# Pixie8888/R3DFSSeg

Measured on AMD Instinct MI355X. Metric: episodes/sec S3DIS 2-way 5-shot 2048-pt (MPTI+attention, train step: forward+backward+grad all-reduce+Adam), higher is better.
Workload: dtype f32 (index-free GEMMs -- self-attention, 1x1 convolutions, weight gradients, the EdgeConv backward's edge GEMMs -- as bf16x3 split products on the bf16 MFMA with fp32 accumulate; every index-deciding result: fp32)

## Files before the change

r3dfsseg_amd/csrc/knn.hip:

```cpp
#include <stdlib.h>
#include "common.h"

#define KNN_Q 32
#define KNN_CH 128
#define KNN_SLAB 64
#define KNN_ROWS_PER_WAVE 8

enum { R3D_SCORE_DGCNN = 0, R3D_SCORE_L2 = 1 };

__global__ void r3d_sqnorm_kernel(const float* __restrict__ x, long ldx, int rows, int C,
                                  float* __restrict__ out) {
  int i = blockIdx.x * blockDim.x + threadIdx.x;
  if (i >= rows) return;
  const float* p = x + (long)i * ldx;
  float acc = 0.f;
  for (int c = 0; c < C; ++c) acc = __builtin_fmaf(p[c], p[c], acc);
  out[i] = acc;
}

template <int R>
struct TopList {
  float v[R];
  int id[R];
};
// ... 342 lines not shown
    const int cbase = 32 * st;
#pragma unroll
    for (int r = 0; r < 16; ++r) {
      const float s_r = sc[r];
      unsigned long long m = __ballot(s_r >= tauq[r] && s_r > thr[r]);
      while (m) {
        unsigned lo = (unsigned)m, hi = (unsigned)(m >> 32);
        const int slo = lo ? __ffs((int)lo) - 1 : 0;
        const int shi = hi ? __ffs((int)hi) - 1 : 0;
        const float cvlo = lo ? r3d_readlane_f(s_r, slo) : -INFINITY;
        const float cvhi = hi ? r3d_readlane_f(s_r, 32 + shi) : -INFINITY;
        lo &= lo - 1;
        hi &= hi - 1;
        m = ((unsigned long long)hi << 32) | lo;
        const float cv = h ? cvhi : cvlo;
        const int cidx = cbase + (h ? shi : slo);
        const bool act = cv > thr[r];
        const unsigned long long ge = __ballot(lv[r] >= cv);
        const int p = h ? __popc((unsigned)(ge >> 32)) : __popc((unsigned)ge);
        const float upv = dpp_wave_shr1_f(lv[r]);
        const int upi = dpp_wave_shr1_i(li[r]);
        if (act) {
          if (j == p) { lv[r] = cv; li[r] = cidx; }
          else if (j > p) { lv[r] = upv; li[r] = upi; }
        }
        const float tlo = r3d_readlane_f(lv[r], klo);
        const float thi = r3d_readlane_f(lv[r], khi);
        thr[r] = h ? thi : tlo;
      }
    }
  };
  {
    int st = w;
    if (st < nsub) bload(st, bfA, njA);
    while (st < nsub) {
      const int st2 = st + 4;
      if (st2 < nsub) bload(st2, bfB, njB);
      {
        f32x16 sc;
        scores(st, bfA, njA, sc);
        select(st, sc);
      }
      st = st2;
      if (st >= nsub) break;
      const int st3 = st + 4;
      if (st3 < nsub) bload(st3, bfA, njA);
      {
        f32x16 sc;
        scores(st, bfB, njB, sc);
        select(st, sc);
      }
      st = st3;
    }
  }
  KSTAMP(3);

  __syncthreads();
  float* mv = smem;
  int* mi = (int*)(smem + 32 * 128);
#pragma unroll
  for (int r = 0; r < 16; ++r) {
    const int q = r3d_acc_row(r, lane);
    mv[(q * 4 + w) * 32 + j] = lv[r];
    mi[(q * 4 + w) * 32 + j] = li[r];
  }
  __syncthreads();
  for (int qq = 0; qq < 8; ++qq) {
    const int q = 8 * w + qq;
    const int row = q0 + q;
    if (row >= n) break;
    const float v0 = mv[q * 128 + lane], v1 = mv[q * 128 + 64 + lane];
    const int i0 = mi[q * 128 + lane], i1 = mi[q * 128 + 64 + lane];
    int rank0 = 0, rank1 = 0;
#pragma unroll
    for (int l4 = 0; l4 < 4; ++l4) {
      const float lvv = (l4 < 2) ? v0 : v1;
      const int lii = (l4 < 2) ? i0 : i1;
      const unsigned long long real = __ballot(lvv != -INFINITY);
      const int cnt = __popc((unsigned)(real >> (32 * (l4 & 1))));
      for (int t = 0; t < cnt; ++t) {
        const float ov = r3d_readlane_f(lvv, 32 * (l4 & 1) + t);
        const int oi = __builtin_amdgcn_readlane(lii, 32 * (l4 & 1) + t);
        rank0 += entry_better(ov, oi, v0, i0) ? 1 : 0;
        rank1 += entry_better(ov, oi, v1, i1) ? 1 : 0;
      }
    }
    if (v0 != -INFINITY && rank0 < k) {
      idx_out[((long)b * N + row) * k + rank0] = i0;
      if (score_out) score_out[((long)b * N + row) * k + rank0] = v0;
    }
    if (v1 != -INFINITY && rank1 < k) {
      idx_out[((long)b * N + row) * k + rank1] = i1;
      if (score_out) score_out[((long)b * N + row) * k + rank1] = v1;
    }
  }
  KSTAMP(4);
}

static __device__ __forceinline__ unsigned knn_lane_xor(unsigned v, int j, int lane) {
  const int x = (int)v;
  switch (j) {
    case 1: return (unsigned)__builtin_amdgcn_update_dpp(x, x, 0xB1, 0xF, 0xF, false);
    case 2: return (unsigned)__builtin_amdgcn_update_dpp(x, x, 0x4E, 0xF, 0xF, false);
    case 4: {
      const int t = __builtin_amdgcn_update_dpp(x, x, 0x104, 0xF, 0x5, false);
      return (unsigned)__builtin_amdgcn_update_dpp(t, x, 0x114, 0xF, 0xA, false);
    }
    case 8: return (unsigned)__builtin_amdgcn_update_dpp(x, x, 0x128, 0xF, 0xF, false);
    case 16: {
      const auto r = __builtin_amdgcn_permlane16_swap(v, v, false, false);
      return (lane & 16) ? r[0] : r[1];
    }
    default: {
      const auto r = __builtin_amdgcn_permlane32_swap(v, v, false, false);
      return (lane & 32) ? r[0] : r[1];
    }
  }
}

template <int R>
static __device__ __forceinline__ void knn_bitonic_desc(unsigned (&khi)[R], unsigned (&klo)[R], int lane) {
  static_assert(R == 1 || R == 2 || R == 4 || R == 8, "a power of two");
#pragma unroll
  for (int k = 2; k <= 64 * R; k <<= 1) {
#pragma unroll
    for (int j = k >> 1; j > 0; j >>= 1) {
      if (j >= 64) {
        const int dj = j >> 6;
#pragma unroll
        for (int i = 0; i < R; ++i) {
          if (i & dj) continue;
          const bool desc = ((64 * i) & k) == 0;
          const unsigned long long a = ((unsigned long long)khi[i] << 32) | klo[i];
          const unsigned long long b = ((unsigned long long)khi[i + dj] << 32) | klo[i + dj];
          const bool swap = desc ? a < b : a > b;
          const unsigned ah = khi[i], al = klo[i];
          khi[i] = swap ? khi[i + dj] : ah; klo[i] = swap ? klo[i + dj] : al;
          khi[i + dj] = swap ? ah : khi[i + dj]; klo[i + dj] = swap ? al : klo[i + dj];
        }
      } else {
        const bool lower = (lane & j) == 0;
#pragma unroll
        for (int i = 0; i < R; ++i) {
          const bool desc = (((64 * i) | lane) & k) == 0;
          const unsigned oh = knn_lane_xor(khi[i], j, lane), ol = knn_lane_xor(klo[i], j, lane);
          const unsigned long long a = ((unsigned long long)khi[i] << 32) | klo[i];
          const unsigned long long b = ((unsigned long long)oh << 32) | ol;
          const bool take = (lower == desc) ? b > a : b < a;
          khi[i] = take ? oh : khi[i];
          klo[i] = take ? ol : klo[i];
        }
      }
    }
  }
}

template <int KB_WAVES, int KB_CAP, int KB_TOP, int KCH ,
          int KB_SAMPLE ,
          bool FULLC ,
          int SMODE ,
          bool BFA ,
          bool BFB = false >
__global__ __launch_bounds__(64 * KB_WAVES) __attribute__((amdgpu_waves_per_eu(KB_WAVES == 4 && (FULLC || KCH < 32) ? 3 : 2)))
void r3d_knn_append_kernel(
    const float* __restrict__ xT, long ldT, int N, int C, int k, int mode, const int* __restrict__ n_dev, int n_dev_stride,
    const float* __restrict__ nrm, int* __restrict__ idx_out, float* __restrict__ score_out,
    int* __restrict__ status, int* __restrict__ tile_flags, int nsplit, int* __restrict__ idx_tmp,
    float* __restrict__ sc_tmp, const unsigned short* __restrict__ xpk ,
    const float* __restrict__ cnorm ,
    const float* __restrict__ xpm , long ldx) {
  static_assert(!BFA || (KCH == 32 && FULLC), "the bf16 threshold pass takes whole 64-channel chunks");
  static_assert(!BFB || BFA, "the bf16 filter pass shares the threshold pass's pieces");
  constexpr int KB_GROUPS = KB_WAVES * 32;
  const int z = blockIdx.z;
  extern __shared__ __attribute__((aligned(16))) float smem[];
  __shared__ int cnt_s[32];
  __shared__ float tau_s[32];
  const int lin = r3d_xcd_swizzle((int)(blockIdx.y * gridDim.x + blockIdx.x), (int)(gridDim.x * gridDim.y));
  const int b = lin / (int)gridDim.x, tile_x = lin - b * (int)gridDim.x;
  const int n = n_dev ? min(n_dev[(long)b * n_dev_stride], N) : N;
  const int q0 = tile_x * 32;
  if (q0 >= n) return;
  const int tid = threadIdx.x, lane = tid & 63, w = tid >> 6;
  const int h = lane >> 5, j = lane & 31;
  const int nch = (C + 2 * KCH - 1) / (2 * KCH);
  const int Cs = nch * 2 * KCH + (BFB ? 4 : 1);
  float* Aq = smem;
  float* region = smem + 32 * Cs;
  const float* xb = xT + (long)b * C * ldT;
  const float* nb = nrm + (long)b * N;

  for (int e = tid; e < 32 * nch * 2 * KCH; e += 64 * KB_WAVES) {
    const int c = e >> 5, jj = e & 31;
    const float v = xb[(long)min(c, C - 1) * ldT + min(q0 + jj, n - 1)];
    Aq[jj * Cs + c] = r3d_keep(v, c < C && q0 + jj < n);
  }
  if (tid < 32) cnt_s[tid] = 0;
  const int Cp = nch * 64;
  const int QRS = 2 * Cp + 8;
  unsigned short* Aqb = reinterpret_cast<unsigned short*>(region + ((32 * (KB_TOP * KB_GROUPS + 1) + 3) & ~3));
  const unsigned short* xpb = BFA ? xpk + (long)b * N * 2 * Cp : nullptr;
  if (BFA) {
    const int cpr = 2 * Cp / 8;
    for (int e = tid; e < 32 * cpr; e += 64 * KB_WAVES) {
      const int c8 = e >> 5, jj = e & 31;
      *reinterpret_cast<r3d_u32x4*>(Aqb + jj * QRS + 8 * c8) =
          *reinterpret_cast<const r3d_u32x4*>(xpb + ((long)c8 * N + min(q0 + jj, n - 1)) * 8);
    }
  }
  KSTAMP(8);
  float nq[16];
#pragma unroll
  for (int r = 0; r < 16; ++r) {
    const int row = q0 + r3d_acc_row(r, lane);
    nq[r] = r3d_keep(nb[min(row, n - 1)], row < n);
  }
  const float* cnb = BFA ? cnorm + (long)b * N : nullptr;
  const float slack = (float)(C + 8) * 0x1p-24f;
  auto bound_k = [&](int i) { return cnb[i] * (1.f + 0x1p-12f) + nb[i] * slack; };
  float* kq_s = reinterpret_cast<float*>(Aqb + 32 * QRS);
  if (BFA && tid < 32) kq_s[tid] = bound_k(min(q0 + tid, n - 1));
  auto bound_ku = [&](int i) { return cnb[i] * (1.f - 0x1p-12f) - nb[i] * slack; };
  if (BFB && tid < 32) kq_s[32 + tid] = bound_ku(min(q0 + tid, n - 1));
  __syncthreads();

  const int nsub = ((n + 31) / 32 - z + nsplit - 1) / nsplit;
  const int my_sub = (nsub - w + KB_WAVES - 1) / KB_WAVES;
  const int T = (w < nsub) ? my_sub * nch : 0;

  int stride = KB_SAMPLE;
  auto bload = [&](int t, float (&bf)[KCH]) {
    const int st = (w + KB_WAVES * stride * (t / nch)) * nsplit + z, ch = (t % nch);
    const int cand = 32 * st + j;
    const bool ok = cand < n;
    const int cc = min(cand, n - 1);
    if (FULLC) {
      const float* p = xb + (long)(2 * KCH * ch + h) * ldT + cc;
      const long st2 = 2 * ldT;
#pragma unroll
      for (int s = 0; s < KCH; ++s) bf[s] = p[s * st2];
    } else {
#pragma unroll
      for (int s = 0; s < KCH; ++s) {
        const int c = 2 * KCH * ch + 2 * s + h;
        bf[s] = r3d_keep(xb[(long)min(c, C - 1) * ldT + cc], ok && c < C);
      }
    }
  };
  f32x16 acc;
  auto mma = [&](int t, const float (&bf)[KCH]) {
    const int ch = (t % nch);
    if (ch == 0) {
#pragma unroll
      for (int r = 0; r < 16; ++r) acc[r] = 0.f;
    }
    const float* ap = Aq + j * Cs + 2 * KCH * ch + h;
    float av[KCH];
#pragma unroll
    for (int s = 0; s < KCH; ++s) av[s] = ap[2 * s];
    __builtin_amdgcn_sched_barrier(0);
#pragma unroll
    for (int s = 0; s < KCH; ++s) acc = __builtin_amdgcn_mfma_f32_32x32x2f32(av[s], bf[s], acc, 0, 0, 0);
  };
  float kb[16];
  auto load_kb = [&](int which) {
#pragma unroll
    for (int r = 0; r < 16; ++r) kb[r] = kq_s[32 * which + r3d_acc_row(r, lane)];
  };
  auto scores_lb = [&](int st, f32x16& sc) {
    const int cand = 32 * st + j;
    const float kj = bound_k(min(cand, n - 1));
#pragma unroll
    for (int r = 0; r < 16; ++r) {
      const float v = __builtin_fmaf(2.f, acc[r], -(kb[r] + kj));
      sc[r] = SMODE == R3D_SCORE_DGCNN ? v : fminf(v, 0.f);
    }
    if (32 * st + 32 > n) {
      const bool valid = cand < n;
#pragma unroll
      for (int r = 0; r < 16; ++r) sc[r] = valid ? sc[r] : -INFINITY;
    }
  };
  auto scores_ub = [&](int st, f32x16& sc) {
    const int cand = 32 * st + j;
    const float kj = bound_ku(min(cand, n - 1));
#pragma unroll
    for (int r = 0; r < 16; ++r) {
      const float v = __builtin_fmaf(2.f, acc[r], -(kb[r] + kj));
      sc[r] = SMODE == R3D_SCORE_DGCNN ? v : fminf(v, 0.f);
    }
    if (32 * st + 32 > n) {
      const bool valid = cand < n;
#pragma unroll
      for (int r = 0; r < 16; ++r) sc[r] = valid ? sc[r] : -INFINITY;
    }
  };
  auto scores = [&](int st, f32x16& sc) {
    const int cand = 32 * st + j;
    const bool valid = cand < n;
    const float nj = r3d_keep(nb[min(cand, n - 1)], valid);
#pragma unroll
    for (int r = 0; r < 16; ++r) {
      float v;
      if (SMODE == R3D_SCORE_DGCNN) {
        const float inner = -2.f * acc[r];
        v = ((-nj) - inner) - nq[r];
// ... 154 lines not shown
  constexpr bool BMP = BFB && KB_WAVES == 4;
  unsigned* bm = reinterpret_cast<unsigned*>(region);
  bool overflow = false;
  auto finishB = [&](int t) {
    if ((t % nch) != nch - 1) return;
    const int st = (w + KB_WAVES * (t / nch)) * nsplit + z;
    f32x16 sc;
    scores(st, sc);
#pragma unroll
    for (int r = 0; r < 16; ++r) {
      if (sc[r] >= tauq[r]) {
        const int q = r3d_acc_row(r, lane);
        const int slot = atomicAdd(&cnt_s[q], 1);
        if (slot < KB_CAP) {
          bufv[q * KB_CAP + slot] = sc[r];
          bufi[q * KB_CAP + slot] = 32 * st + j;
        } else {
          overflow = true;
        }
      }
    }
  };
  auto finishBF = [&](int i) {
    const int st = (w + KB_WAVES * i) * nsplit + z;
    f32x16 sc;
    scores_ub(st, sc);
    if (BMP) {
      unsigned long long m[16];
#pragma unroll
      for (int r = 0; r < 16; ++r) m[r] = __ballot(sc[r] >= tauq[r]);
      __builtin_amdgcn_sched_barrier(0);
      int word = 0;
#define KB_LO(r) "s"((int)(unsigned)(m[r] & 0xffffffffull))
#define KB_HI(r) "s"((int)(unsigned)(m[r] >> 32))
      asm volatile(
                   "s_nop 4\n\t"
                   "v_writelane_b32 %0, %1, 0\n\t"
                   "v_writelane_b32 %0, %2, 4\n\t"
                   "v_writelane_b32 %0, %3, 1\n\t"
                   "v_writelane_b32 %0, %4, 5\n\t"
                   "v_writelane_b32 %0, %5, 2\n\t"
                   "v_writelane_b32 %0, %6, 6\n\t"
                   "v_writelane_b32 %0, %7, 3\n\t"
                   "v_writelane_b32 %0, %8, 7\n\t"
                   "v_writelane_b32 %0, %9, 8\n\t"
                   "v_writelane_b32 %0, %10, 12\n\t"
                   "v_writelane_b32 %0, %11, 9\n\t"
                   "v_writelane_b32 %0, %12, 13\n\t"
                   "v_writelane_b32 %0, %13, 10\n\t"
                   "v_writelane_b32 %0, %14, 14\n\t"
                   "v_writelane_b32 %0, %15, 11\n\t"
                   "v_writelane_b32 %0, %16, 15"
                   : "+v"(word)
                   : KB_LO(0), KB_HI(0), KB_LO(1), KB_HI(1), KB_LO(2), KB_HI(2), KB_LO(3), KB_HI(3), KB_LO(4), KB_HI(4), KB_LO(5), KB_HI(5), KB_LO(6), KB_HI(6), KB_LO(7), KB_HI(7));
      asm volatile(
                   "s_nop 4\n\t"
                   "v_writelane_b32 %0, %1, 16\n\t"
                   "v_writelane_b32 %0, %2, 20\n\t"
                   "v_writelane_b32 %0, %3, 17\n\t"
                   "v_writelane_b32 %0, %4, 21\n\t"
                   "v_writelane_b32 %0, %5, 18\n\t"
                   "v_writelane_b32 %0, %6, 22\n\t"
                   "v_writelane_b32 %0, %7, 19\n\t"
                   "v_writelane_b32 %0, %8, 23\n\t"
                   "v_writelane_b32 %0, %9, 24\n\t"
                   "v_writelane_b32 %0, %10, 28\n\t"
                   "v_writelane_b32 %0, %11, 25\n\t"
                   "v_writelane_b32 %0, %12, 29\n\t"
                   "v_writelane_b32 %0, %13, 26\n\t"
                   "v_writelane_b32 %0, %14, 30\n\t"
                   "v_writelane_b32 %0, %15, 27\n\t"
                   "v_writelane_b32 %0, %16, 31"
                   : "+v"(word)
                   : KB_LO(8), KB_HI(8), KB_LO(9), KB_HI(9), KB_LO(10), KB_HI(10), KB_LO(11), KB_HI(11), KB_LO(12), KB_HI(12), KB_LO(13), KB_HI(13), KB_LO(14), KB_HI(14), KB_LO(15), KB_HI(15));
#undef KB_LO
#undef KB_HI
      __builtin_amdgcn_sched_barrier(0);
      const int ls = w + KB_WAVES * i;
      if (lane < 32) bm[ls * 32 + ((lane + ls) & 31)] = (unsigned)word;
      return;
    }
#pragma unroll
    for (int r = 0; r < 16; ++r) {
      if (sc[r] >= tauq[r]) {
        const int q = r3d_acc_row(r, lane);
        const int slot = atomicAdd(&cnt_s[q], 1);
        if (slot < KB_CAP) bufi[q * KB_CAP + slot] = 32 * st + j;
        else overflow = true;
      }
    }
  };
  if (BFB) {
    load_kb(1);
    bf_pass((w < nsub) ? my_sub : 0, finishBF);
  } else {
    if (T > 0) bload(0, bfB);
    for (int t = 0; t < T; ++t) {
#pragma unroll
      for (int s = 0; s < KCH; ++s) bfA[s] = bfB[s];
      if (t + 1 < T) bload(t + 1, bfB);
      __builtin_amdgcn_sched_barrier(0);
      mma(t, bfA);
      finishB(t);
    }
  }
  KSTAMP(12);
  if (BMP) {
    __syncthreads();
    constexpr int QW = 32 / KB_WAVES, NCH = (KB_CAP + 63) / 64;
    unsigned wq[QW][NCH];
#pragma unroll
    for (int i = 0; i < QW; ++i)
#pragma unroll
      for (int cch = 0; cch < NCH; ++cch) {
        const int ls = 64 * cch + lane;
        wq[i][cch] = ls < nsub ? bm[ls * 32 + ((QW * w + i + ls) & 31)] : 0u;
      }
    __syncthreads();
#pragma unroll
    for (int i = 0; i < QW; ++i) {
      const int q = QW * w + i;
      int total = 0;
#pragma unroll
      for (int cch = 0; cch < NCH; ++cch) {
        if (64 * cch >= nsub) break;
        unsigned word = wq[i][cch];
        const int c = __popc(word);
        const int incl = r3d_wave_incl_scan(c);
        int off = total + incl - c;
        const int cand0 = 32 * ((64 * cch + lane) * nsplit + z);
        while (word) {
          const int bit = __ffs((int)word) - 1;
          if (off < KB_CAP) bufi[q * KB_CAP + off] = cand0 + bit;
          ++off;
          word &= word - 1;
        }
        total += __builtin_amdgcn_readlane(incl, 63);
      }
      if (lane == 0) cnt_s[q] = total;
      overflow = overflow || total > KB_CAP;
    }
  }
  if (__any(overflow) && lane == 0) {
    if (status) atomicOr(status, 1);
    if (tile_flags) tile_flags[(long)b * gridDim.x + tile_x] = 1;
  }
  __syncthreads();
  if (BFA && tid < 32 && q0 + tid < n && cnt_s[tid] < min(k, n)) {
    if (status) atomicOr(status, 2);
    if (tile_flags) tile_flags[(long)b * gridDim.x + tile_x] = 1;
  }
  KSTAMP(14);

  if (BFB) {
    constexpr int QW = 32 / KB_WAVES;
    int off[QW + 1];
    off[0] = 0;
#pragma unroll
    for (int i = 0; i < QW; ++i) off[i + 1] = off[i] + __builtin_amdgcn_readfirstlane(min(cnt_s[QW * w + i], KB_CAP));
    const int total = off[QW];
    const int nseg = C / 32;
    const int T2 = ((total + 63) / 64) * nseg;
    int q_cur = 0, slot_cur = 0;
    bool ok_cur = false;
    const float4* xr_cur = nullptr;
    auto locate = [&](int t, int& q, int& slot, bool& ok, const float4*& xr) {
      const int f = 64 * (t / nseg) + lane;
      ok = f < total;
      int ql = 0;
#pragma unroll
      for (int i = 1; i < QW; ++i) ql += f >= off[i] ? 1 : 0;
      ql = ok ? ql : 0;
      q = QW * w + ql;
      slot = ok ? f - off[ql] : 0;
      const int cand = min(max(bufi[q * KB_CAP + slot], 0), n - 1);
      xr = reinterpret_cast<const float4*>(xpm + ((long)b * N + cand) * ldx) + 8 * (t % nseg);
    };
    float4 xa[8], xb[8];
    int qn = 0, slotn = 0;
    bool okn = false;
    const float4* xrn = nullptr;
    if (T2 > 0) {
      locate(0, q_cur, slot_cur, ok_cur, xr_cur);
#pragma unroll
      for (int u = 0; u < 8; ++u) xa[u] = xr_cur[u];
    }
    float a = 0.f;
    for (int t = 0; t < T2; ++t) {
      const int tn = min(t + 1, T2 - 1);
      locate(tn, qn, slotn, okn, xrn);
#pragma unroll
      for (int u = 0; u < 8; ++u) xb[u] = xrn[u];
      __builtin_amdgcn_sched_barrier(0);
      const int sg = t % nseg;
      if (sg == 0) a = 0.f;
      const float4* aq = reinterpret_cast<const float4*>(Aq + q_cur * Cs + 32 * sg);
      float4 qa[8];
#pragma unroll
      for (int u = 0; u < 8; ++u) qa[u] = aq[u];
#pragma unroll
      for (int u = 0; u < 8; ++u) {
        a = __builtin_fmaf(qa[u].x, xa[u].x, a);
        a = __builtin_fmaf(qa[u].y, xa[u].y, a);
        a = __builtin_fmaf(qa[u].z, xa[u].z, a);
        a = __builtin_fmaf(qa[u].w, xa[u].w, a);
      }
      if (sg == nseg - 1 && ok_cur) {
        const int cand = min(max(bufi[q_cur * KB_CAP + slot_cur], 0), n - 1);
        const float nj = nb[cand], nqq = nb[min(q0 + q_cur, n - 1)];
        float v;
        if (SMODE == R3D_SCORE_DGCNN) {
          const float inner = -2.f * a;
          v = ((-nj) - inner) - nqq;
        } else {
          const float dis = (nqq + nj) - 2.f * a;
          v = -fmaxf(dis, 0.f);
        }
        bufv[q_cur * KB_CAP + slot_cur] = v;
      }
#pragma unroll
      for (int u = 0; u < 8; ++u) xa[u] = xb[u];
      q_cur = qn; slot_cur = slotn; ok_cur = okn;
    }
  }
  KSTAMP(15);
  for (int qq = 0; qq < 32 / KB_WAVES; ++qq) {
    const int q = (32 / KB_WAVES) * w + qq;
    const int row = q0 + q;
    if (row >= n) break;
    const int M = __builtin_amdgcn_readfirstlane(min(cnt_s[q], KB_CAP));
    float mv[KB_CAP / 64];
    int mi[KB_CAP / 64], rank[KB_CAP / 64];
    unsigned khi[KB_CAP / 64], klo[KB_CAP / 64];
    unsigned long long key[KB_CAP / 64];
#pragma unroll
    for (int i = 0; i < KB_CAP / 64; ++i) {
      const int e = 64 * i + lane;
      mi[i] = e < M ? bufi[q * KB_CAP + e] : 0x7fffffff;
      mv[i] = e < M ? bufv[q * KB_CAP + e] : -INFINITY;
      khi[i] = f2key(mv[i] + 0.0f);
      klo[i] = 0x7fffffffu - (unsigned)mi[i];
      key[i] = ((unsigned long long)khi[i] << 32) | klo[i];
      rank[i] = 0;
    }
    bool sorted = false;
    if constexpr (KB_CAP >= 256) {
    if (M > 64 && N <= (1 << 22)) {
      constexpr int RMAX = KB_CAP > 256 ? 8 : 4;
      static_assert(64 * RMAX >= KB_CAP && KB_CAP <= 512, "the slot field of a sort key has 9 bits");
      unsigned sh[RMAX], sl[RMAX];
#pragma unroll
      for (int i = 0; i < RMAX; ++i) {
        const int e = 64 * i + lane;
        const bool in = i < KB_CAP / 64 && e < M;
        sh[i] = in ? khi[i < KB_CAP / 64 ? i : 0] : 0u;
        sl[i] = in ? ((0x3fffffu - (unsigned)mi[i < KB_CAP / 64 ? i : 0]) << 9) | (unsigned)e : 0u;
      }
      if (M <= 256) {
        unsigned h4[4] = {sh[0], sh[1], sh[2], sh[3]}, l4[4] = {sl[0], sl[1], sl[2], sl[3]};
        knn_bitonic_desc<4>(h4, l4, lane);
#pragma unroll
        for (int i = 0; i < 4; ++i) sl[i] = l4[i];
      } else {
        knn_bitonic_desc<RMAX>(sh, sl, lane);
      }
#pragma unroll
      for (int i = 0; i < KB_CAP / 64; ++i) {
        const int e = 64 * i + lane;
        const int slot = (int)(sl[i] & 511u);
        const bool out = e < M;
        mi[i] = out ? bufi[q * KB_CAP + slot] : 0x7fffffff;
        mv[i] = out ? bufv[q * KB_CAP + slot] : -INFINITY;
        rank[i] = e;
      }
      sorted = true;
    }
    }
    if (sorted) {
    } else if (M <= 64) {
#pragma unroll 4
      for (int t = 0; t < M; ++t) {
        const unsigned long long ok = ((unsigned long long)(unsigned)__builtin_amdgcn_readlane((int)khi[0], t) << 32) |
                                      (unsigned)__builtin_amdgcn_readlane((int)klo[0], t);
        rank[0] += ok > key[0] ? 1 : 0;
      }
    } else {
#pragma unroll
      for (int c = 0; c < KB_CAP / 64; ++c) {
        const int cnt = min(max(M - 64 * c, 0), 64);
#pragma unroll 4
        for (int t = 0; t < cnt; ++t) {
          const unsigned long long ok = ((unsigned long long)(unsigned)__builtin_amdgcn_readlane((int)khi[c], t) << 32) |
                                        (unsigned)__builtin_amdgcn_readlane((int)klo[c], t);
#pragma unroll
          for (int i = 0; i < KB_CAP / 64; ++i) rank[i] += ok > key[i] ? 1 : 0;
        }
      }
    }
    if (nsplit == 1) {
#pragma unroll
      for (int i = 0; i < KB_CAP / 64; ++i) {
        if (64 * i + lane < M && rank[i] < k) {
          idx_out[((long)b * N + row) * k + rank[i]] = mi[i];
          if (score_out) score_out[((long)b * N + row) * k + rank[i]] = mv[i];
        }
      }
    } else {
      const long o = (((long)z * gridDim.y + b) * N + row) * k;
#pragma unroll
      for (int i = 0; i < KB_CAP / 64; ++i) {
        if (64 * i + lane < M && rank[i] < k) {
          idx_tmp[o + rank[i]] = mi[i];
          sc_tmp[o + rank[i]] = mv[i];
        }
      }
      for (int t = min(M, k) + lane; t < k; t += 64) {
        idx_tmp[o + t] = 0x7fffffff;
        sc_tmp[o + t] = -INFINITY;
      }
    }
  }
  KSTAMP(13);
}

__global__ __launch_bounds__(256) void r3d_knn_merge_kernel(const int* __restrict__ idx_tmp, const float* __restrict__ sc_tmp,
                                                            int nsplit, long rows, int k, const int* __restrict__ n_dev, int n_dev_stride, int N,
                                                            int* __restrict__ idx_out, float* __restrict__ score_out) {
  __shared__ unsigned long long keys[4][2][256];
  const int lane = threadIdx.x & 63, w = threadIdx.x >> 6;
  const long row = (long)blockIdx.x * 4 + w;
  if (row >= rows) return;
  if (n_dev && (int)(row % N) >= min(n_dev[(row / N) * n_dev_stride], N)) return;
  for (int p = 0; p < 2; ++p)
    for (int t = lane; t < k; t += 64) {
      const long o = ((long)p * rows + row) * k + t;
      const float v = sc_tmp[o];
      const int id = idx_tmp[o];
      keys[w][p][t] = id == 0x7fffffff ? 0ull
                                       : (((unsigned long long)f2key(v + 0.0f) << 32) | (0x7fffffffu - (unsigned)id));
    }
  __builtin_amdgcn_wave_barrier();
  for (int p = 0; p < 2; ++p)
    for (int t = lane; t < k; t += 64) {
      const unsigned long long mine = keys[w][p][t];
      if (mine == 0ull) continue;
      const unsigned long long* other = keys[w][1 - p];
      int lo = 0, hi = k;
      while (lo < hi) {
        const int mid = (lo + hi) >> 1;
        if (other[mid] > mine) lo = mid + 1; else hi = mid;
      }
      const int rank = t + lo;
      if (rank < k) {
        const long o = ((long)p * rows + row) * k + t;
        idx_out[row * k + rank] = idx_tmp[o];
        if (score_out) score_out[row * k + rank] = sc_tmp[o];
      }
    }
}

__global__ __launch_bounds__(1024) void r3d_knn_mean_kernel(const float* __restrict__ x, long ldx, int N, int C,
                                                            const int* __restrict__ n_dev, int n_dev_stride, int Cp,
                                                            float* __restrict__ mean ) {
  __shared__ float part[16][64];
  const int b = blockIdx.y, c = blockIdx.x * 64 + (threadIdx.x & 63), ph = threadIdx.x >> 6;
  const int n = n_dev ? min(n_dev[(long)b * n_dev_stride], N) : N;
  float s = 0.f;
  if (c < C) {
    const float* p = x + (long)b * N * ldx + c;
    int r = ph;
    for (; r + 7 * 16 < n; r += 8 * 16) {
      float v[8];
#pragma unroll
      for (int u = 0; u < 8; ++u) v[u] = p[(long)(r + 16 * u) * ldx];
#pragma unroll
      for (int u = 0; u < 8; ++u) s += v[u];
    }
    for (; r < n; r += 16) s += p[(long)r * ldx];
  }
  part[ph][threadIdx.x & 63] = s;
  __syncthreads();
  if (ph == 0 && c < Cp) {
    float t = 0.f;
#pragma unroll
    for (int q = 0; q < 16; ++q) t += part[q][threadIdx.x];
    mean[(long)b * Cp + c] = c < C && n > 0 ? t / (float)n : 0.f;
  }
}
__global__ void r3d_knn_pack_bf_kernel(const float* __restrict__ x, long ldx, long rows, int N, int C, int Cp,
                                       const float* __restrict__ mean, unsigned short* __restrict__ out) {
  const long i = (long)blockIdx.x * blockDim.x + threadIdx.x;
  const int cpr = Cp / 8;
  if (i >= rows * cpr) return;
  const long m = i / cpr;
  const int c8 = (int)(i - m * cpr);
  const long set = m / N;
  const int pt = (int)(m - set * N);
  const int c0 = 8 * c8;
  const float* mu = mean + set * Cp + c0;
  float v[8];
#pragma unroll
  for (int u = 0; u < 8; ++u) v[u] = r3d_keep(x[m * ldx + min(c0 + u, C - 1)] - mu[u], c0 + u < C);
  const r3d_bx3 f = r3d_bx3_split8(v);
  unsigned short* o = out + set * N * 2 * Cp;
  *reinterpret_cast<r3d_u32x4*>(o + ((long)c8 * N + pt) * 8) = f.h;
  *reinterpret_cast<r3d_u32x4*>(o + ((long)(cpr + c8) * N + pt) * 8) = f.m;
}
__global__ __launch_bounds__(256) void r3d_knn_cnorm_kernel(const float* __restrict__ x, long ldx, long rows, int N, int C, int Cp,
                                                            const float* __restrict__ mean, float* __restrict__ cnorm) {
  const int lane = threadIdx.x & 63, sub = lane & 15;
  const long m = ((long)blockIdx.x * 4 + (threadIdx.x >> 6)) * 4 + (lane >> 4);
  const long mc = m < rows ? m : rows - 1;
  const float* mu = mean + (mc / N) * Cp;
  float s = 0.f;
  if ((ldx & 3) == 0 && (C & 3) == 0 && ((uintptr_t)x & 15) == 0) {
    for (int c = 4 * sub; c < C; c += 64) {
      const float4 v = *reinterpret_cast<const float4*>(x + mc * ldx + c), u = *reinterpret_cast<const float4*>(mu + c);
      const float d0 = v.x - u.x, d1 = v.y - u.y, d2 = v.z - u.z, d3 = v.w - u.w;
      s = __builtin_fmaf(d0, d0, s); s = __builtin_fmaf(d1, d1, s); s = __builtin_fmaf(d2, d2, s); s = __builtin_fmaf(d3, d3, s);
    }
  } else {
    for (int c = sub; c < C; c += 16) {
      const float d = x[mc * ldx + c] - mu[c];
      s = __builtin_fmaf(d, d, s);
    }
  }
  s += __int_as_float(__builtin_amdgcn_mov_dpp(__float_as_int(s), 0xB1, 0xF, 0xF, true));
  s += __int_as_float(__builtin_amdgcn_mov_dpp(__float_as_int(s), 0x4E, 0xF, 0xF, true));
  s += __int_as_float(__builtin_amdgcn_mov_dpp(__float_as_int(s), 0x141, 0xF, 0xF, true));
  s += __int_as_float(__builtin_amdgcn_mov_dpp(__float_as_int(s), 0x140, 0xF, 0xF, true));
  if (sub == 0 && m < rows) cnorm[m] = s;
}
static int g_knn_bf16_threshold = getenv("R3D_KNN_FP32_THRESHOLD") ? 0 : 1;
static int g_knn_bf16_filter = getenv("R3D_KNN_FP32_PASS_B") ? 0 : 1;
extern "C" int r3d_debug_set_knn_bf16_filter(int on) {
  const int old = g_knn_bf16_filter;
  g_knn_bf16_filter = on > 0 ? 1 : 0;
  return old;
}
extern "C" int r3d_debug_set_knn_bf16_threshold(int on) {
  const int old = g_knn_bf16_threshold;
  g_knn_bf16_threshold = on ? 1 : 0;
  return old;
}
#ifndef KM_WAVES
#define KM_WAVES 4
#define KM_CAP 128
#define KM_TOP 1
#endif
#ifndef KM_SAMPLE
#define KM_SAMPLE 2
#endif

static size_t knn_append_lds_bytes(int C, int waves, int cap, int top, int kch, bool bfa) {
  const int nch = (C + 2 * kch - 1) / (2 * kch);
  const size_t a = 32 * (size_t)(nch * 2 * kch + 4);
  size_t g = 32 * (size_t)(top * waves * 32 + 1);
  if (bfa) g = ((g + 3) & ~(size_t)3) + 32 * (size_t)(2 * nch * 64 + 8) / 2 + 64;
  const size_t bsz = 2 * 32 * (size_t)cap;
  return sizeof(float) * (a + (g > bsz ? g : bsz));
}
static size_t knn_lds_bytes(int C) {
  const int Cp = (C + 1) & ~1;
  return sizeof(float) * ((size_t)KNN_Q * (Cp + 1) + (size_t)KNN_CH * (KNN_SLAB + 1) +
                          (size_t)KNN_Q * (KNN_CH + 1) + KNN_Q);
}

static int knn_sqnorm_launch(const float* x, long ldx, long rows, int C, float* out, void* stream) {
  R3D_REQUIRE(x && out && rows > 0 && C > 0 && ldx >= C, "r3d_sqnorm: bad arguments");
  hipLaunchKernelGGL(r3d_sqnorm_kernel, dim3(r3d_cdiv(rows, 256)), dim3(256), 0, (hipStream_t)stream, x,
                     ldx, (int)rows, C, out);
  R3D_LAUNCH_CHECK("r3d_sqnorm");
  return R3D_OK;
}

extern "C" long r3d_cm_pitch(int N) { return (long)((N + 31) / 32) * 32 + 32; }
extern "C" long r3d_knn_norm_ws_words(int B, int N) { return (long)B * N + (long)B * ((N + 31) / 32) + 64; }

enum KnnPath {
  KNN_STREAMED_SMALL,
  KNN_STREAMED_LARGE,
  KNN_INSERTION,
};
struct KnnPlan {
  KnnPath path;
  bool few;
  bool split;
  bool bf;
  long norms, tile_flags, xcm, pieces, mean, cnorm, split_idx, split_sc, words;
};
static KnnPlan knn_plan(int B, int N, int C, int k, bool status, bool x_cm, bool extras) {
  KnnPlan p = {};
  const long tiles = ((long)N + 31) / 32;
  if (k <= 32 && C <= 64) {
    p.path = KNN_STREAMED_SMALL;
    p.few = tiles * B <= 256;
    p.bf = extras && C % 64 == 0 && !p.few;
  } else if (status && knn_append_lds_bytes(C, 8, 384, 2, 32, false) <= 160 * 1024) {
    p.path = KNN_STREAMED_LARGE;
    p.split = extras && 2 * tiles * B <= 256 && N >= 4L * k;
    p.bf = extras && !p.split && C % 64 == 0 && knn_append_lds_bytes(C, 8, 384, 2, 32, true) <= 160 * 1024;
  } else {
    p.path = KNN_INSERTION;
  }
  long at = 0;
  auto part = [&](long words) {
    const long o = at;
    at += (words + 63) / 64 * 64;
    return o;
  };
  p.norms = part((long)B * N);
  p.tile_flags = part(p.path == KNN_STREAMED_SMALL ? B * tiles : 0);
  p.xcm = part(p.path != KNN_INSERTION && !x_cm ? (long)B * C * r3d_cm_pitch(N) : 0);
  p.pieces = part(p.bf ? (long)B * N * C : 0);
  p.mean = part(p.bf ? (long)B * C : 0);
  p.cnorm = part(p.bf ? (long)B * N : 0);
  p.split_idx = part(p.split ? 2L * B * N * k : 0);
  p.split_sc = part(p.split ? 2L * B * N * k : 0);
  p.words = at;
  return p;
}

extern "C" long r3d_knn_ws_words(int B, int N, int C, int k, int flags) {
  return knn_plan(B, N, C, k, flags & 1, flags & 2, true).words;
}

struct KnnCall {
  const float* x; long ldx; const float* xT; long ldT;
  int B, N, C, k, mode; const int* n_dev; int n_stride; int32_t* idx; float* sc; hipStream_t st;
  float *norms; int* tile_flags; float* cm; unsigned short* pieces; float *mean, *cnorm; int* split_idx; float* split_sc;
};

template <int WAVES, int CAP, int TOP, int KCH, int SAMPLE, bool FULLC, bool BFA = false, bool BFB = false>
static int knn_append_launch(const KnnCall& c, dim3 grid, int* status, int* tile_flags) {
  const size_t lds = knn_append_lds_bytes(c.C, WAVES, CAP, TOP, KCH, BFA);
  auto go = [&](auto smode) {
    constexpr int SM = decltype(smode)::value;
    static size_t attr = 0;
    if (lds > attr) {
      hipError_t e = hipFuncSetAttribute((const void*)r3d_knn_append_kernel<WAVES, CAP, TOP, KCH, SAMPLE, FULLC, SM, BFA, BFB>,
                                         hipFuncAttributeMaxDynamicSharedMemorySize, (int)lds);
      R3D_REQUIRE(e == hipSuccess, "r3d_knn_topk: cannot reserve %zu B of LDS: %s", lds, hipGetErrorString(e));
      attr = lds;
    }
    hipLaunchKernelGGL((r3d_knn_append_kernel<WAVES, CAP, TOP, KCH, SAMPLE, FULLC, SM, BFA, BFB>), grid, dim3(64 * WAVES), lds,
                       c.st, c.xT, c.ldT, c.N, c.C, c.k, SM, c.n_dev, c.n_stride, c.norms, c.idx, c.sc, status, tile_flags,
                       (int)grid.z, c.split_idx, c.split_sc, BFA ? c.pieces : nullptr, BFA ? c.cnorm : nullptr,
                       BFB ? c.x : nullptr, c.ldx);
    return R3D_OK;
  };
  return c.mode == R3D_SCORE_DGCNN ? go(std::integral_constant<int, R3D_SCORE_DGCNN>())
                                   : go(std::integral_constant<int, R3D_SCORE_L2>());
}

template <int R>
static void knn_insertion_launch(const KnnCall& c, size_t lds) {
  static bool attr_set = false;
  if (!attr_set) {
    hipFuncSetAttribute((const void*)r3d_knn_topk_kernel<R>, hipFuncAttributeMaxDynamicSharedMemorySize, 160 * 1024);
    attr_set = true;
  }
  hipLaunchKernelGGL(r3d_knn_topk_kernel<R>, dim3(r3d_cdiv(c.N, KNN_Q), c.B), dim3(256), lds, c.st, c.x, c.ldx, c.N, c.C,
                     c.k, c.mode, c.n_dev, c.n_stride, c.norms, c.idx, c.sc);
}

static int knn_cm_operand(KnnCall& c, const float* x_cm) {
  c.xT = x_cm;
  c.ldT = c.N;
  if (!x_cm) {
    R3D_REQUIRE(c.cm && c.x, "r3d_knn_topk: need x_cm or (x and cm_ws)");
    c.ldT = r3d_cm_pitch(c.N);
    int rc = r3d_pm_to_cm_pitched_launch(c.x, c.ldx, c.B, c.C, c.N, c.cm, c.ldT, c.st);
    if (rc) return rc;
    c.xT = c.cm;
  }
  hipLaunchKernelGGL(r3d_sqnorm_cm_kernel, dim3(r3d_cdiv(c.N, 256), c.B), dim3(256), 0, c.st, c.xT, c.ldT, c.C, c.N, c.norms);
  return R3D_OK;
}

static void knn_pack_bf(const KnnCall& c) {
  const long rows = (long)c.B * c.N;
  hipLaunchKernelGGL(r3d_knn_mean_kernel, dim3(c.C / 64, c.B), dim3(1024), 0, c.st, c.x, c.ldx, c.N, c.C, c.n_dev, c.n_stride,
                     c.C, c.mean);
  hipLaunchKernelGGL(r3d_knn_pack_bf_kernel, dim3(r3d_cdiv(rows * (c.C / 8), 256)), dim3(256), 0, c.st, c.x, c.ldx, rows, c.N,
                     c.C, c.C, c.mean, c.pieces);
  hipLaunchKernelGGL(r3d_knn_cnorm_kernel, dim3(r3d_cdiv(rows, 16)), dim3(256), 0, c.st, c.x, c.ldx, rows, c.N, c.C, c.C,
                     c.mean, c.cnorm);
}

static int knn_topk_impl(const float* x, long ldx, const float* x_cm, int B, int N, int C, int k, int mode,
                         const int* n_valid_dev, int n_valid_stride, float* ws, long ws_words, float* norm_ws, float* cm_ws,
                         int32_t* idx_out, float* score_out, int32_t* status, void* stream) {
  R3D_REQUIRE((x || x_cm) && (ws || norm_ws) && idx_out, "r3d_knn_topk: null pointer");
  R3D_REQUIRE(B > 0 && N > 0 && C > 0 && (!x || ldx >= C), "r3d_knn_topk: bad shape B=%d N=%d C=%d ldx=%ld", B, N, C, ldx);
  R3D_REQUIRE(k > 0 && k <= N && k <= 256, "r3d_knn_topk: unsupported k=%d (need 1..min(N,256))", k);
  R3D_REQUIRE(mode == R3D_SCORE_DGCNN || mode == R3D_SCORE_L2, "r3d_knn_topk: unknown mode %d", mode);
  const KnnPlan p = knn_plan(B, N, C, k, status, x_cm, ws);
  KnnCall c = {x, ldx, nullptr, 0, B, N, C, k, mode, n_valid_dev, n_valid_stride, idx_out, score_out, (hipStream_t)stream};
  if (ws) {
    R3D_REQUIRE(((uintptr_t)ws & 15) == 0 && ws_words >= p.words,
                "r3d_knn_topk_batched: ws must be 16-byte aligned and hold r3d_knn_ws_words = %ld floats (got %ld)", p.words,
                ws_words);
    c.norms = ws + p.norms;
    c.tile_flags = (int*)(ws + p.tile_flags);
    c.cm = ws + p.xcm;
    c.pieces = (unsigned short*)(ws + p.pieces);
    c.mean = ws + p.mean;
    c.cnorm = ws + p.cnorm;
    c.split_idx = (int*)(ws + p.split_idx);
    c.split_sc = ws + p.split_sc;
  } else {
    c.norms = norm_ws;
    c.tile_flags = (int*)(norm_ws + (long)B * N);
    c.cm = cm_ws;
  }
  if (p.path == KNN_INSERTION) {
    R3D_REQUIRE(c.x, "r3d_knn_topk: the insertion kernel needs the point-major matrix");
    const size_t lds = knn_lds_bytes(c.C);
    R3D_REQUIRE(lds <= 160 * 1024, "r3d_knn_topk: C=%d needs %zu B of LDS (> 160 KiB)", c.C, lds);
    int rc = knn_sqnorm_launch(c.x, c.ldx, (long)c.B * c.N, c.C, c.norms, c.st);
    if (rc) return rc;
    if (c.k <= 64) knn_insertion_launch<1>(c, lds);
    else if (c.k <= 128) knn_insertion_launch<2>(c, lds);
    else knn_insertion_launch<4>(c, lds);
    R3D_LAUNCH_CHECK("r3d_knn_topk");
    return R3D_OK;
  }
  int rc = knn_cm_operand(c, x_cm);
  if (rc) return rc;
  const bool bfa = p.bf && g_knn_bf16_threshold && c.x;
  const dim3 grid(r3d_cdiv(c.N, 32), c.B);
  if (p.path == KNN_STREAMED_SMALL) {
    r3d_zero_words(c.tile_flags, (long)c.B * grid.x, c.st);
    if (c.C <= 16) {
      rc = p.few ? knn_append_launch<8, KM_CAP, KM_TOP, 8, KM_SAMPLE, false>(c, grid, nullptr, c.tile_flags)
                 : knn_append_launch<KM_WAVES, KM_CAP, KM_TOP, 8, KM_SAMPLE, false>(c, grid, nullptr, c.tile_flags);
    } else if (bfa) {
      knn_pack_bf(c);
      const bool filter = g_knn_bf16_filter && (c.ldx & 3) == 0 && ((uintptr_t)c.x & 15) == 0 && grid.x <= KM_CAP;
      rc = filter ? knn_append_launch<KM_WAVES, KM_CAP, KM_TOP, 32, 1, true, true, true>(c, grid, nullptr, c.tile_flags)
                  : knn_append_launch<KM_WAVES, KM_CAP, KM_TOP, 32, KM_SAMPLE, true, true>(c, grid, nullptr, c.tile_flags);
    } else if (c.C % 64 == 0) {
      rc = p.few ? knn_append_launch<8, KM_CAP, KM_TOP, 32, KM_SAMPLE, true>(c, grid, nullptr, c.tile_flags)
                 : knn_append_launch<KM_WAVES, KM_CAP, KM_TOP, 32, KM_SAMPLE, true>(c, grid, nullptr, c.tile_flags);
    } else {
      rc = p.few ? knn_append_launch<8, KM_CAP, KM_TOP, 32, KM_SAMPLE, false>(c, grid, nullptr, c.tile_flags)
                 : knn_append_launch<KM_WAVES, KM_CAP, KM_TOP, 32, KM_SAMPLE, false>(c, grid, nullptr, c.tile_flags);
    }
    if (rc) return rc;
    hipLaunchKernelGGL(c.C <= 16 ? r3d_knn_small_kernel<8> : r3d_knn_small_kernel<32>, grid, dim3(256), 0, c.st, c.xT, c.ldT, c.N,
                       c.C, c.k, c.mode, c.n_dev, c.n_stride, c.norms, c.idx, c.sc, (const int*)c.tile_flags);
    R3D_LAUNCH_CHECK("r3d_knn_topk(small)");
    return R3D_OK;
  }
  r3d_zero_words(status, 1, c.st);
  const dim3 gb(grid.x, c.B, p.split ? 2 : 1);
  if (bfa) {
    knn_pack_bf(c);
    rc = knn_append_launch<8, 384, 2, 32, 1, true, true>(c, gb, status, nullptr);
  } else if (c.C % 64 == 0) {
    rc = knn_append_launch<8, 384, 2, 32, 1, true>(c, gb, status, nullptr);
  } else {
    rc = knn_append_launch<8, 384, 2, 32, 1, false>(c, gb, status, nullptr);
  }
  if (rc) return rc;
  if (p.split)
    hipLaunchKernelGGL(r3d_knn_merge_kernel, dim3(r3d_cdiv((long)c.B * c.N, 4)), dim3(256), 0, c.st, c.split_idx, c.split_sc, 2,
                       (long)c.B * c.N, c.k, c.n_dev, c.n_stride, c.N, c.idx, c.sc);
  R3D_LAUNCH_CHECK("r3d_knn_topk(big)");
  return R3D_OK;
}

extern "C" int r3d_knn_topk(const float* x, long ldx, const float* x_cm, int B, int N, int C, int k, int mode,
                            const int* n_valid_dev, float* norm_ws, float* cm_ws, int32_t* idx_out,
                            float* score_out, int32_t* status, void* stream) {
  return knn_topk_impl(x, ldx, x_cm, B, N, C, k, mode, n_valid_dev, 0, nullptr, 0, norm_ws, cm_ws, idx_out, score_out, status,
                       stream);
}

extern "C" int r3d_knn_topk_batched(const float* x, long ldx, const float* x_cm, int B, int N, int C, int k, int mode,
                                    const int* n_valid_dev, int n_valid_stride, float* ws, long ws_words, int32_t* idx_out,
                                    float* score_out, int32_t* status, void* stream) {
  R3D_REQUIRE(n_valid_stride >= 0, "r3d_knn_topk_batched: negative stride");
  return knn_topk_impl(x, ldx, x_cm, B, N, C, k, mode, n_valid_dev, n_valid_stride, ws, ws_words, nullptr, nullptr, idx_out,
                       score_out, status, stream);
}
```

Before: 387.2.

## Stage candidate rows through LDS for exact KNN rescoring and enable on big path

Rewrites the exact fp32 rescoring pass of the bf16-filtered KNN so each wave loads candidate feature rows cooperatively with coalesced float4 loads into LDS (reusing the wave's score slots plus extra LDS) and then computes dot products from LDS, with software prefetch of the next slab. Scores are kept in registers and written back at the end so the score buffer can double as staging space. The default filter level becomes 2, which switches the large-N path to this BFB variant when alignment, no-split and LDS limits allow. This adds LDS pressure and wave-level fences, and the default is now a new pass on the big path.

Measured after the change: 392.3, median of 6. 1.3% higher.

```diff
diff --git a/r3dfsseg_amd/csrc/knn.hip b/r3dfsseg_amd/csrc/knn.hip
--- a/r3dfsseg_amd/csrc/knn.hip
+++ b/r3dfsseg_amd/csrc/knn.hip
@@ -518,6 +518,154 @@
         }
       }
     }
+  }
+}
+
+#define KNN_XS_SLAB 32
+#define KNN_XS_PITCH (KNN_XS_SLAB + 4)
+constexpr int knn_xs_rows(int waves) { return waves == 4 ? 32 : 64; }
+constexpr int knn_xs_rows_lo(int waves, int cap) {
+  const int fit = ((32 / waves) * cap / KNN_XS_PITCH) / 8 * 8;
+  return fit < knn_xs_rows(waves) ? fit : knn_xs_rows(waves);
+}
+constexpr int knn_xs_extra_floats(int waves, int cap) {
+  return waves * (knn_xs_rows(waves) - knn_xs_rows_lo(waves, cap)) * KNN_XS_PITCH;
+}
+
+template <int KB_WAVES, int KB_CAP, int SMODE>
+static __device__ __forceinline__ void knn_exact_scores(
+    const float* __restrict__ xrows , long ldx, int C ,
+    int n, const float* __restrict__ nb , int q0, const float* Aq ,
+    int Cs , const int* bufi , float* bufv ,
+    const int* cnt_s , float* xs_extra , int w, int lane) {
+  constexpr int QW = 32 / KB_WAVES;
+  constexpr int P = KNN_XS_PITCH;
+  constexpr int RS = knn_xs_rows(KB_WAVES);
+  constexpr int HALVES = 64 / RS;
+  constexpr int R0 = knn_xs_rows_lo(KB_WAVES, KB_CAP);
+  constexpr int NI = RS / 8;
+  constexpr int NB = QW * KB_CAP / 64;
+  static_assert(R0 % 8 == 0 && R0 * P <= QW * KB_CAP && (QW * KB_CAP) % 64 == 0, "staging rows inside the wave's score slots");
+  int off[QW + 1];
+  off[0] = 0;
+#pragma unroll
+  for (int i = 0; i < QW; ++i) off[i + 1] = off[i] + __builtin_amdgcn_readfirstlane(min(cnt_s[QW * w + i], KB_CAP));
+  const int total = off[QW];
+  if (total == 0) return;
+  const int nbatch = (total + 63) / 64, nslab = C / KNN_XS_SLAB;
+  float* lo = bufv + QW * w * KB_CAP;
+  float* hi = xs_extra + w * ((RS - R0) * P);
+  auto locate = [&](int bt, int& q, int& slot, bool& ok) {
+    const int f = 64 * bt + lane;
+    ok = f < total;
+    int ql = 0;
+#pragma unroll
+    for (int i = 1; i < QW; ++i) ql += f >= off[i] ? 1 : 0;
+    ql = ok ? ql : 0;
+    q = QW * w + ql;
+    slot = ok ? f - off[ql] : 0;
+  };
+  const float* rp[8];
+  auto rows_of = [&](int cand) {
+#pragma unroll
+    for (int g = 0; g < 8; ++g) rp[g] = xrows + (long)__shfl(cand, 8 * g + (lane >> 3)) * ldx + 4 * (lane & 7);
+  };
+  auto fetch = [&](f32x4 (&pf)[NI], int hf , int s) {
+#pragma unroll
+    for (int i = 0; i < NI; ++i) pf[i] = *reinterpret_cast<const f32x4*>(rp[hf * NI + i] + KNN_XS_SLAB * s);
+  };
+  auto stage = [&](const f32x4 (&pf)[NI]) {
+#pragma unroll
+    for (int i = 0; i < NI; ++i) {
+      const int r = 8 * i + (lane >> 3);
+      float* d = 8 * i < R0 ? lo + r * P : hi + (r - R0) * P;
+      *reinterpret_cast<f32x4*>(d + 4 * (lane & 7)) = pf[i];
+    }
+  };
+  const int myr = lane % RS;
+  const float* myrow = myr < R0 ? lo + myr * P : hi + (myr - R0) * P;
+  auto wave_lds_order = [&]() {
+    __builtin_amdgcn_fence(__ATOMIC_ACQ_REL, "wavefront");
+    __builtin_amdgcn_wave_barrier();
+  };
+
+  int q_c, slot_c, cand_c;
+  bool ok_c;
+  locate(0, q_c, slot_c, ok_c);
+  cand_c = min(max(bufi[q_c * KB_CAP + slot_c], 0), n - 1);
+  rows_of(cand_c);
+  f32x4 pf[NI];
+  fetch(pf, 0, 0);
+  float keep[NB];
+#pragma unroll
+  for (int i = 0; i < NB; ++i) keep[i] = 0.f;
+  float a = 0.f;
+  for (int bt = 0; bt < nbatch; ++bt) {
+    const float* aqrow = Aq + q_c * Cs;
+    int q_n = q_c, slot_n = slot_c, cand_n = cand_c;
+    bool ok_n = ok_c;
+    for (int s = 0; s < nslab; ++s) {
+      if (s == 0) a = 0.f;
+#pragma unroll
+      for (int hf = 0; hf < HALVES; ++hf) {
+        wave_lds_order();
+        stage(pf);
+        if (hf + 1 < HALVES) {
+          fetch(pf, hf + 1, s);
+        } else {
+          int s_n = s + 1;
+          if (s_n == nslab) {
+            if (bt + 1 < nbatch) {
+              s_n = 0;
+              locate(bt + 1, q_n, slot_n, ok_n);
+              cand_n = min(max(bufi[q_n * KB_CAP + slot_n], 0), n - 1);
+              rows_of(cand_n);
+            } else {
+              s_n = s;
+            }
+          }
+          fetch(pf, 0, s_n);
+        }
+        __builtin_amdgcn_sched_barrier(0);
+        wave_lds_order();
+        if (HALVES == 1 || (lane / RS) == hf) {
+          const f32x4* xr = reinterpret_cast<const f32x4*>(myrow);
+          const f32x4* aq = reinterpret_cast<const f32x4*>(aqrow + KNN_XS_SLAB * s);
+          f32x4 xa[8], qa[8];
+#pragma unroll
+          for (int u = 0; u < 8; ++u) { xa[u] = xr[u]; qa[u] = aq[u]; }
+#pragma unroll
+          for (int u = 0; u < 8; ++u) {
+            a = __builtin_fmaf(qa[u].x, xa[u].x, a);
+            a = __builtin_fmaf(qa[u].y, xa[u].y, a);
+            a = __builtin_fmaf(qa[u].z, xa[u].z, a);
+            a = __builtin_fmaf(qa[u].w, xa[u].w, a);
+          }
+        }
+      }
+    }
+    {
+      const float nj = nb[cand_c], nqq = nb[min(q0 + q_c, n - 1)];
+      float v;
+      if (SMODE == R3D_SCORE_DGCNN) {
+        const float inner = -2.f * a;
+        v = ((-nj) - inner) - nqq;
+      } else {
+        const float dis = (nqq + nj) - 2.f * a;
+        v = -fmaxf(dis, 0.f);
+      }
+#pragma unroll
+      for (int i = 0; i < NB; ++i) keep[i] = bt == i ? v : keep[i];
+    }
+    q_c = q_n; slot_c = slot_n; cand_c = cand_n; ok_c = ok_n;
+  }
+  wave_lds_order();
+#pragma unroll
+  for (int i = 0; i < NB; ++i) {
+    int q, slot;
+    bool ok;
+    locate(i, q, slot, ok);
+    if (ok) bufv[q * KB_CAP + slot] = keep[i];
   }
 }
 
@@ -978,76 +1126,10 @@
   }
   KSTAMP(14);
 
-  if (BFB) {
-    constexpr int QW = 32 / KB_WAVES;
-    int off[QW + 1];
-    off[0] = 0;
-#pragma unroll
-    for (int i = 0; i < QW; ++i) off[i + 1] = off[i] + __builtin_amdgcn_readfirstlane(min(cnt_s[QW * w + i], KB_CAP));
-    const int total = off[QW];
-    const int nseg = C / 32;
-    const int T2 = ((total + 63) / 64) * nseg;
-    int q_cur = 0, slot_cur = 0;
-    bool ok_cur = false;
-    const float4* xr_cur = nullptr;
-    auto locate = [&](int t, int& q, int& slot, bool& ok, const float4*& xr) {
-      const int f = 64 * (t / nseg) + lane;
-      ok = f < total;
-      int ql = 0;
-#pragma unroll
-      for (int i = 1; i < QW; ++i) ql += f >= off[i] ? 1 : 0;
-      ql = ok ? ql : 0;
-      q = QW * w + ql;
-      slot = ok ? f - off[ql] : 0;
-      const int cand = min(max(bufi[q * KB_CAP + slot], 0), n - 1);
-      xr = reinterpret_cast<const float4*>(xpm + ((long)b * N + cand) * ldx) + 8 * (t % nseg);
-    };
-    float4 xa[8], xb[8];
-    int qn = 0, slotn = 0;
-    bool okn = false;
-    const float4* xrn = nullptr;
-    if (T2 > 0) {
-      locate(0, q_cur, slot_cur, ok_cur, xr_cur);
-#pragma unroll
-      for (int u = 0; u < 8; ++u) xa[u] = xr_cur[u];
-    }
-    float a = 0.f;
-    for (int t = 0; t < T2; ++t) {
-      const int tn = min(t + 1, T2 - 1);
-      locate(tn, qn, slotn, okn, xrn);
-#pragma unroll
-      for (int u = 0; u < 8; ++u) xb[u] = xrn[u];
-      __builtin_amdgcn_sched_barrier(0);
-      const int sg = t % nseg;
-      if (sg == 0) a = 0.f;
-      const float4* aq = reinterpret_cast<const float4*>(Aq + q_cur * Cs + 32 * sg);
-      float4 qa[8];
-#pragma unroll
-      for (int u = 0; u < 8; ++u) qa[u] = aq[u];
-#pragma unroll
-      for (int u = 0; u < 8; ++u) {
-        a = __builtin_fmaf(qa[u].x, xa[u].x, a);
-        a = __builtin_fmaf(qa[u].y, xa[u].y, a);
-        a = __builtin_fmaf(qa[u].z, xa[u].z, a);
-        a = __builtin_fmaf(qa[u].w, xa[u].w, a);
-      }
-      if (sg == nseg - 1 && ok_cur) {
-        const int cand = min(max(bufi[q_cur * KB_CAP + slot_cur], 0), n - 1);
-        const float nj = nb[cand], nqq = nb[min(q0 + q_cur, n - 1)];
-        float v;
-        if (SMODE == R3D_SCORE_DGCNN) {
-          const float inner = -2.f * a;
-          v = ((-nj) - inner) - nqq;
-        } else {
-          const float dis = (nqq + nj) - 2.f * a;
-          v = -fmaxf(dis, 0.f);
-        }
-        bufv[q_cur * KB_CAP + slot_cur] = v;
-      }
-#pragma unroll
-      for (int u = 0; u < 8; ++u) xa[u] = xb[u];
-      q_cur = qn; slot_cur = slotn; ok_cur = okn;
-    }
+  if constexpr (BFB) {
+    float* xs_extra = kq_s + 64 > region + 64 * KB_CAP ? kq_s + 64 : region + 64 * KB_CAP;
+    knn_exact_scores<KB_WAVES, KB_CAP, SMODE>(xpm + (long)b * N * ldx, ldx, C, n, nb, q0, Aq, Cs, bufi, bufv, cnt_s, xs_extra, w,
+                                              lane);
   }
   KSTAMP(15);
   for (int qq = 0; qq < 32 / KB_WAVES; ++qq) {
@@ -1258,10 +1340,10 @@
   if (sub == 0 && m < rows) cnorm[m] = s;
 }
 static int g_knn_bf16_threshold = getenv("R3D_KNN_FP32_THRESHOLD") ? 0 : 1;
-static int g_knn_bf16_filter = getenv("R3D_KNN_FP32_PASS_B") ? 0 : 1;
+static int g_knn_bf16_filter = getenv("R3D_KNN_FP32_PASS_B") ? 0 : 2;
 extern "C" int r3d_debug_set_knn_bf16_filter(int on) {
   const int old = g_knn_bf16_filter;
-  g_knn_bf16_filter = on > 0 ? 1 : 0;
+  g_knn_bf16_filter = on < 0 ? 0 : on > 2 ? 2 : on;
   return old;
 }
 extern "C" int r3d_debug_set_knn_bf16_threshold(int on) {
@@ -1278,13 +1360,14 @@
 #define KM_SAMPLE 2
 #endif
 
-static size_t knn_append_lds_bytes(int C, int waves, int cap, int top, int kch, bool bfa) {
+static size_t knn_append_lds_bytes(int C, int waves, int cap, int top, int kch, bool bfa, bool bfb = false) {
   const int nch = (C + 2 * kch - 1) / (2 * kch);
   const size_t a = 32 * (size_t)(nch * 2 * kch + 4);
   size_t g = 32 * (size_t)(top * waves * 32 + 1);
   if (bfa) g = ((g + 3) & ~(size_t)3) + 32 * (size_t)(2 * nch * 64 + 8) / 2 + 64;
   const size_t bsz = 2 * 32 * (size_t)cap;
-  return sizeof(float) * (a + (g > bsz ? g : bsz));
+  const size_t xs = bfb ? knn_xs_extra_floats(waves, cap) : 0;
+  return sizeof(float) * (a + (g > bsz ? g : bsz) + xs);
 }
 static size_t knn_lds_bytes(int C) {
   const int Cp = (C + 1) & ~1;
@@ -1359,7 +1442,7 @@
 
 template <int WAVES, int CAP, int TOP, int KCH, int SAMPLE, bool FULLC, bool BFA = false, bool BFB = false>
 static int knn_append_launch(const KnnCall& c, dim3 grid, int* status, int* tile_flags) {
-  const size_t lds = knn_append_lds_bytes(c.C, WAVES, CAP, TOP, KCH, BFA);
+  const size_t lds = knn_append_lds_bytes(c.C, WAVES, CAP, TOP, KCH, BFA, BFB);
   auto go = [&](auto smode) {
     constexpr int SM = decltype(smode)::value;
     static size_t attr = 0;
@@ -1483,7 +1566,10 @@
   const dim3 gb(grid.x, c.B, p.split ? 2 : 1);
   if (bfa) {
     knn_pack_bf(c);
-    rc = knn_append_launch<8, 384, 2, 32, 1, true, true>(c, gb, status, nullptr);
+    const bool filter = g_knn_bf16_filter >= 2 && !p.split && (c.ldx & 3) == 0 && ((uintptr_t)c.x & 15) == 0 &&
+                        knn_append_lds_bytes(c.C, 8, 384, 2, 32, true, true) <= 160 * 1024;
+    rc = filter ? knn_append_launch<8, 384, 2, 32, 1, true, true, true>(c, gb, status, nullptr)
+                : knn_append_launch<8, 384, 2, 32, 1, true, true>(c, gb, status, nullptr);
   } else if (c.C % 64 == 0) {
     rc = knn_append_launch<8, 384, 2, 32, 1, true>(c, gb, status, nullptr);
   } else {
```
